# IlzeAmandaA/VAE-GP-ODE

Measured on AMD Instinct MI355X. Metric: latent_trajectories_per_sec, higher is better.
Workload: dtype f32; 1 GPU; configs[1]: ode1 DF q=6 M=100 S=256 T=16 batch=256; step = full ELBO training step (encoder, GP draw, rk4 rollout, decoder, ELBO, backward, Adam), L=1; global_batch=256, mc_draws=1, solver=rk4 (3/8 rule), parallelism=dp1, hip_graph=True, graph_scope=whole, gp_side_stream=True, batchnorm=per-process statistics

## Files before the change

vae-gp-ode_amd/csrc/gp_backward.hip:

```cpp
#include "gp_rollout.hpp"

namespace gp {

template <int DI, int DO, int NJ>
__device__ __forceinline__ void store_grads_rbf(const typename RbfTeamEval<DI, DO, NJ>::Grads& G, float* __restrict__ out, int M, int S,
                                                int wave, int lane, float (*sInd)[64][4 * RbfLayout<DI, DO>::RQ2],
                                                float (*sUni)[((DO + 1) / 2) * DI]);
template <int D, int NJ, int PART = 0>
__device__ __forceinline__ void store_grads_df(const typename DfTeamEval<D, NJ>::Grads& G, float* __restrict__ out, int M, int S, int wave,
                                               int lane, float (*sInd)[64][4 * DfLayout<D>::RQ2],
                                               float (*sUni)[2 * D * ((D + 1) / 2) + (D + 1) / 2]);

template <class EV, bool PG> struct GradsOf { using type = NoGrads; };
template <class EV> struct GradsOf<EV, true> { using type = typename EV::Grads; };

template <class EV, int DI, int DO, int ORDER, int METHOD, bool PG = false, bool SUB = false>
__global__ __launch_bounds__(64 * EV::kTeam) void rollout_bwd_team_kernel(const float* __restrict__ pack, int M, int S,
                                                                const float* __restrict__ xstage, const float* __restrict__ gzt,
                                                                const float* __restrict__ ts, int N, int T,
                                                                float* __restrict__ gz0, float* __restrict__ astage, Draws dw,
                                                                float* __restrict__ slab = nullptr, size_t pack_floats = 0) {
  constexpr int NS = stages_of(METHOD);
  __shared__ float slots[2 * EV::kTeam * TeamCombine::DP];
  pack += blockIdx.y * dw.pack; xstage += blockIdx.y * dw.in; gzt += blockIdx.y * dw.in2; gz0 += blockIdx.y * dw.out; astage += blockIdx.y * dw.out2;
  const int lane = threadIdx.x & 63, wave = threadIdx.x >> 6;
  EV ev;
  ev.init(pack, M, S, slots, wave, lane);
  using GR = typename GradsOf<EV, PG>::type;
  GR G;
  if constexpr (PG) G.zero();
  const float third = (float)(1.0 / 3.0);
  const int sub = sub_count<SUB>(dw.sub);
  for (int n = blockIdx.x; n < N; n += gridDim.x) {
    const float* gz = gzt + (size_t)n * T * DI;
    const float* xs = xstage + (size_t)n * (T - 1) * sub * NS * DI;
    float* as = astage + (size_t)n * (T - 1) * sub * NS * DO;
    float lam[DI];
#pragma unroll
    for (int i = 0; i < DI; ++i) lam[i] = gz[(size_t)(T - 1) * DI + i];
    const float* tn = ts_row(ts, n, dw.ts);
    for (int t = T - 2; t >= 0; --t) {
      const float dt = sub_step<SUB>(tn[t], tn[t + 1], sub);
      for (int r = (t + 1) * sub - 1; r >= t * sub; --r) {
        const float* xt = xs + (size_t)r * NS * DI;
        float* at = as + (size_t)r * NS * DO;
        float x[DI], g[DI], af[DO];
        if (METHOD == 0) {
          float a1[DI];
#pragma unroll
          for (int i = 0; i < DI; ++i) { a1[i] = dt * lam[i]; x[i] = xt[i]; }
          ode_vjp<EV, DI, DO, ORDER, GR>(ev, x, a1, g, af, &G);
          if (wave == 0) store_state<DO>(at, af, lane);
#pragma unroll
          for (int i = 0; i < DI; ++i) lam[i] += g[i];
        } else if (METHOD == 2) {
          float a1[DI], a2[DI], ay[DI];
#pragma unroll
          for (int i = 0; i < DI; ++i) { a2[i] = dt * lam[i]; x[i] = xt[DI + i]; }
          ode_vjp<EV, DI, DO, ORDER, GR>(ev, x, a2, g, af, &G);
          if (wave == 0) store_state<DO>(at + DO, af, lane);
#pragma unroll
          for (int i = 0; i < DI; ++i) { ay[i] = lam[i] + g[i]; a1[i] = 0.5f * dt * g[i]; x[i] = xt[i]; }
          ode_vjp<EV, DI, DO, ORDER, GR>(ev, x, a1, g, af, &G);
          if (wave == 0) store_state<DO>(at, af, lane);
#pragma unroll
          for (int i = 0; i < DI; ++i) lam[i] = ay[i] + g[i];
        } else {
          float a1[DI], a2[DI], a3[DI], a4[DI], ay[DI];
#pragma unroll
          for (int i = 0; i < DI; ++i) {
            const float l8 = lam[i] * dt * 0.125f;
            a1[i] = l8; a4[i] = l8; a2[i] = 3.f * l8; a3[i] = 3.f * l8; ay[i] = lam[i];
          }
#pragma unroll
          for (int i = 0; i < DI; ++i) x[i] = xt[3 * DI + i];
          ode_vjp<EV, DI, DO, ORDER, GR>(ev, x, a4, g, af, &G);
          if (wave == 0) store_state<DO>(at + 3 * DO, af, lane);
#pragma unroll
          for (int i = 0; i < DI; ++i) { ay[i] += g[i]; a1[i] += dt * g[i]; a2[i] -= dt * g[i]; a3[i] += dt * g[i]; }
#pragma unroll
          for (int i = 0; i < DI; ++i) x[i] = xt[2 * DI + i];
          ode_vjp<EV, DI, DO, ORDER, GR>(ev, x, a3, g, af, &G);
// ... 176 lines not shown
    float red[NU];
    wave_sum_all<NU>(flat, red);
    if (lane == 0) {
#pragma unroll
      for (int e = 0; e < NU; ++e) sUni[wave][e] = red[e];
    }
  }
  __syncthreads();
  if (half == 0 && j < MJ) {
    float* ind_out = out + 4 * L::rff_f4(S);
    float v[4 * L::RQ2];
#pragma unroll
    for (int q = 0; q < 4 * L::RQ2; ++q) v[q] = G.ind[q] + sInd[j][lane][q];
#pragma unroll
    for (int q = 0; q < L::RQ2; ++q) st4(ind_out, (size_t)(j * L::RQ2 + q) * 64 + lane, &v[4 * q]);
  }
  {
    float* uni_out = out + 4 * (L::rff_f4(S) + L::ind_f4(M));
    const int t = threadIdx.x;
    if (t < D * D) {
      const int a = t / D, b = t % D, h = b / DH, bb = b % DH;
      uni_out[a * D + b] = sUni[h][a * DH + bb] + sUni[h + 2][a * DH + bb];
      uni_out[D * D + a * D + b] = sUni[h][D * DH + a * DH + bb] + sUni[h + 2][D * DH + a * DH + bb];
    }
    if (t < D) {
      const int h = t / DH, bb = t % DH;
      uni_out[2 * D * D + t] = sUni[h][2 * D * DH + bb] + sUni[h + 2][2 * D * DH + bb];
    }
  }
}

template <int D, int NJ>
__global__ __launch_bounds__(256) void param_grad_df_kernel(const float* __restrict__ pack, int M, int S,
                                                             const float* __restrict__ xr, const float* __restrict__ ar,
                                                             int R, int rows_per_chunk, float* __restrict__ slab,
                                                             size_t pack_floats, int prior_only, Draws dw, int slab_chunks) {
  pack += blockIdx.y * dw.pack; xr += blockIdx.y * dw.in; ar += blockIdx.y * dw.in2; slab += (size_t)blockIdx.y * slab_chunks * pack_floats;
  using EV = DfTeamEval<D, NJ>;
  using L = DfLayout<D>;
  constexpr int DH = (D + 1) / 2;
  constexpr int NU = 2 * D * DH + DH;
  __shared__ float slots[2 * TEAM * TeamCombine::DP];
  __shared__ __attribute__((aligned(16))) float sInd[2][64][4 * L::RQ2];
  __shared__ float sUni[TEAM][NU];
  const int lane = threadIdx.x & 63, wave = threadIdx.x >> 6;
  EV ev;
  ev.init(pack, M, S, slots, wave, lane);
  typename EV::Grads G;
  G.zero();
  const int r0 = blockIdx.x * rows_per_chunk;
  const int r1 = min(R, r0 + rows_per_chunk);
  for (int r = r0; r < r1; ++r) {
    float x[D], a[D];
#pragma unroll
    for (int i = 0; i < D; ++i) { x[i] = xr[(size_t)r * D + i]; a[i] = ar[(size_t)r * D + i]; }
    ev.grad_row(x, a, G, prior_only != 0);
  }
  store_grads_df<D, NJ>(G, slab + (size_t)blockIdx.x * pack_floats, M, S, wave, lane, sInd, sUni);
}

template <int D, int PART>
__device__ __forceinline__ void pgrad_df_part(const float* __restrict__ pack, int M, int S, const float* __restrict__ xr,
                                              const float* __restrict__ ar, int r0, int r1, float* __restrict__ out, int prior_only) {
  using EV = DfTeamEval<D, 1>;
  using L = DfLayout<D>;
  constexpr int DH = (D + 1) / 2;
  constexpr int NU = 2 * D * DH + DH;
  __shared__ float slots[2 * TEAM * TeamCombine::DP];
  __shared__ __attribute__((aligned(16))) float sInd[2][64][4 * L::RQ2];
  __shared__ float sUni[TEAM][NU];
  const int lane = threadIdx.x & 63, wave = threadIdx.x >> 6;
  EV ev;
  ev.init(pack, M, S, slots, wave, lane);
  typename EV::Grads G;
  G.zero();
  for (int r = r0; r < r1; ++r) {
    float x[D], a[D];
#pragma unroll
    for (int i = 0; i < D; ++i) { x[i] = xr[(size_t)r * D + i]; a[i] = ar[(size_t)r * D + i]; }
    ev.template grad_row_part<PART>(x, a, G, prior_only != 0);
  }
  store_grads_df<D, 1, PART>(G, out, M, S, wave, lane, sInd, sUni);
}
template <int D>
__global__ __launch_bounds__(256, 2) void param_grad_df_split_kernel(const float* __restrict__ pack, int M, int S,
                                                                      const float* __restrict__ xr, const float* __restrict__ ar,
                                                                      int R, int rows_per_chunk, float* __restrict__ slab,
                                                                      size_t pack_floats, int prior_only, Draws dw, int slab_chunks) {
  pack += blockIdx.y * dw.pack; xr += blockIdx.y * dw.in; ar += blockIdx.y * dw.in2; slab += (size_t)blockIdx.y * slab_chunks * pack_floats;
  const int r0 = blockIdx.x * rows_per_chunk, r1 = min(R, r0 + rows_per_chunk);
  float* out = slab + (size_t)blockIdx.x * pack_floats;
  if (blockIdx.z == 0) pgrad_df_part<D, 1>(pack, M, S, xr, ar, r0, r1, out, prior_only);
  else pgrad_df_part<D, 2>(pack, M, S, xr, ar, r0, r1, out, prior_only);
}

template <int DI, int DO>
__global__ __launch_bounds__(256) void param_grad_rbf_stream_kernel(const float* __restrict__ pack, int M, int S,
                                                                     const float* __restrict__ xr, const float* __restrict__ ar,
                                                                     int R, int rows_per_chunk, float* __restrict__ slab,
                                                                     size_t pack_floats, int prior_only, Draws dw, int slab_chunks) {
  pack += blockIdx.y * dw.pack; xr += blockIdx.y * dw.in; ar += blockIdx.y * dw.in2; slab += (size_t)blockIdx.y * slab_chunks * pack_floats;
  using L = RbfLayout<DI, DO>;
  constexpr int DH = (DO + 1) / 2;
  __shared__ __attribute__((aligned(16))) float sInd[2][64][4 * L::RQ2];
  __shared__ float sUni[TEAM][DH * DI];
  const int lane = threadIdx.x & 63, wave = __builtin_amdgcn_readfirstlane(threadIdx.x >> 6);
  const float4* p4 = reinterpret_cast<const float4*>(pack);
  const float4* i4 = p4 + L::rff_f4(S);
  const float* wl = pack + 4 * (L::rff_f4(S) + L::ind_f4(M));
  const int r0 = blockIdx.x * rows_per_chunk, r1 = min(R, r0 + rows_per_chunk);
  float* out = slab + (size_t)blockIdx.x * pack_floats;
  const int SJ = cdiv(S, 64), MJ = cdiv(M, 64);
  for (int rec = wave; rec < SJ * DO; rec += TEAM) {
    float4 rq[L::RQ];
    load_record<L::RQ>(p4, rec, lane, rq);
    float g[4 * L::RQ];
#pragma unroll
    for (int q = 0; q < 4 * L::RQ; ++q) g[q] = 0.f;
    const int d = rec % DO;
    for (int r = r0; r < r1; ++r) {
      float x[DI], gx[DI];
#pragma unroll
      for (int i = 0; i < DI; ++i) { x[i] = xr[(size_t)r * DI + i]; gx[i] = 0.f; }
      rbf_rff_bwd<DI, DO, true>(rq, x, ar[(size_t)r * DO + d], gx, g);
    }
#pragma unroll
    for (int q = 0; q < L::RQ; ++q) st4(out, ((size_t)rec * L::RQ + q) * 64 + lane, &g[4 * q]);
  }
  const int half = wave & 1;
  float gwl[DH][DI];
#pragma unroll
  for (int d = 0; d < DH; ++d)
#pragma unroll
    for (int i = 0; i < DI; ++i) gwl[d][i] = 0.f;
  float* ind_out = out + 4 * L::rff_f4(S);
  for (int jb = 0; jb < MJ; jb += 2) {
    const int j = jb + (wave >> 1);
    const bool valid = j < MJ;
    float4 ind[L::RQ2];
    float gi[4 * L::RQ2];
#pragma unroll
    for (int q = 0; q < 4 * L::RQ2; ++q) gi[q] = 0.f;
    if (valid) {
      load_record<L::RQ2>(i4, j, lane, ind);
      if (!prior_only) {
        for (int r = r0; r < r1; ++r) {
          asm volatile("" ::: "memory");
          float x[DI], a[DO], gx[DI];
#pragma unroll
          for (int i = 0; i < DI; ++i) { x[i] = xr[(size_t)r * DI + i]; gx[i] = 0.f; }
#pragma unroll
          for (int i = 0; i < DO; ++i) a[i] = ar[(size_t)r * DO + i];
          rbf_ind_half_bwd<DI, DO, true>(ind, x, wl, half, a, gx, gi, gwl);
        }
      }
    }
    if (half == 1) {
#pragma unroll
      for (int q = 0; q < 4 * L::RQ2; ++q) sInd[wave >> 1][lane][q] = gi[q];
    }
    __syncthreads();
    if (half == 0 && valid) {
      float v[4 * L::RQ2];
#pragma unroll
      for (int q = 0; q < 4 * L::RQ2; ++q) v[q] = gi[q] + sInd[wave >> 1][lane][q];
#pragma unroll
      for (int q = 0; q < L::RQ2; ++q) st4(ind_out, ((size_t)j * L::RQ2 + q) * 64 + lane, &v[4 * q]);
    }
    __syncthreads();
  }
  {
    float flat[DH * DI], red[DH * DI];
#pragma unroll
    for (int e = 0; e < DH * DI; ++e) flat[e] = gwl[e / DI][e % DI];
    wave_sum_all<DH * DI>(flat, red);
    if (lane == 0) {
// ... 46 lines not shown
    for (int q = 0; q < L::RQ; ++q) st4(out, ((size_t)rec * L::RQ + q) * 64 + lane, &g[4 * q]);
  }
  const int part = wave % NP, slot = wave / NP;
  float gwab[D][DQ], gil2[D][DQ], gvar[DQ];
#pragma unroll
  for (int a = 0; a < D; ++a)
#pragma unroll
    for (int b = 0; b < DQ; ++b) { gwab[a][b] = 0.f; gil2[a][b] = 0.f; }
#pragma unroll
  for (int b = 0; b < DQ; ++b) gvar[b] = 0.f;
  float* ind_out = out + 4 * L::rff_f4(S);
  for (int jb = 0; jb < MJ; jb += RPI) {
    const int j = jb + slot;
    const bool valid = j < MJ;
    float4 ind[L::RQ2];
    float gi[4 * L::RQ2];
#pragma unroll
    for (int q = 0; q < 4 * L::RQ2; ++q) gi[q] = 0.f;
    if (valid) {
      load_record<L::RQ2>(i4, j, lane, ind);
      if (!prior_only) {
        for (int r = r0; r < r1; ++r) {
          asm volatile("" ::: "memory");
          float x[D], a[D], gx[D];
#pragma unroll
          for (int i = 0; i < D; ++i) { x[i] = xr[(size_t)r * D + i]; a[i] = ar[(size_t)r * D + i]; gx[i] = 0.f; }
          df_ind_part_bwd<D, NP, true>(ind, x, uni, part, a, gx, gi, gwab, gil2, gvar);
        }
      }
    }
    if (part > 0) {
#pragma unroll
      for (int q = 0; q < 4 * L::RQ2; ++q) sInd[slot][part - 1][lane][q] = gi[q];
    }
    __syncthreads();
    if (part == 0 && valid) {
      float v[4 * L::RQ2];
#pragma unroll
      for (int q = 0; q < 4 * L::RQ2; ++q) {
        v[q] = gi[q];
#pragma unroll
        for (int pp = 0; pp < NP - 1; ++pp) v[q] += sInd[slot][pp][lane][q];
      }
#pragma unroll
      for (int q = 0; q < L::RQ2; ++q) st4(ind_out, ((size_t)j * L::RQ2 + q) * 64 + lane, &v[4 * q]);
    }
    __syncthreads();
  }
  {
    float flat[NU];
#pragma unroll
    for (int a = 0; a < D; ++a)
#pragma unroll
      for (int b = 0; b < DQ; ++b) { flat[a * DQ + b] = gwab[a][b]; flat[D * DQ + a * DQ + b] = gil2[a][b]; }
#pragma unroll
    for (int b = 0; b < DQ; ++b) flat[2 * D * DQ + b] = gvar[b];
    float red[NU];
    wave_sum_all<NU>(flat, red);
    if (lane == 0) {
#pragma unroll
      for (int e = 0; e < NU; ++e) sUni[wave][e] = red[e];
    }
  }
  __syncthreads();
  {
    float* uni_out = out + 4 * (L::rff_f4(S) + L::ind_f4(M));
    for (int t = threadIdx.x; t < D * D; t += 256) {
      const int a = t / D, b = t % D, pt = b / DQ, bb = b % DQ;
      float v0 = 0.f, v1 = 0.f;
      for (int w = pt; w < TEAM; w += NP) { v0 += sUni[w][a * DQ + bb]; v1 += sUni[w][D * DQ + a * DQ + bb]; }
      uni_out[a * D + b] = v0;
      uni_out[D * D + a * D + b] = v1;
    }
    if (threadIdx.x < D) {
      const int t = threadIdx.x, pt = t / DQ, bb = t % DQ;
      float v = 0.f;
      for (int w = pt; w < TEAM; w += NP) v += sUni[w][2 * D * DQ + bb];
      uni_out[2 * D * D + t] = v;
    }
  }
}

__global__ __launch_bounds__(1024) void reduce_slab_kernel(const float* __restrict__ slab, int nchunk, size_t pack_floats,
                                                            float* __restrict__ gpack, int accumulate, size_t gpack_dstride, int slab_chunks) {
  __shared__ float red[16][64];
  slab += (size_t)blockIdx.y * slab_chunks * pack_floats; gpack += blockIdx.y * gpack_dstride;
  const int ex = threadIdx.x & 63, cg = threadIdx.x >> 6;
  const size_t e = (size_t)blockIdx.x * 64 + ex;
  float acc = 0.f;
  if (e < pack_floats) {
#pragma unroll 8
    for (int c = cg; c < nchunk; c += 16) acc += slab[(size_t)c * pack_floats + e];
  }
  red[cg][ex] = acc;
  __syncthreads();
  if (cg == 0 && e < pack_floats) {
    float v = accumulate ? gpack[e] : 0.f;
#pragma unroll
    for (int g = 0; g < 16; ++g) v += red[g][ex];
    gpack[e] = v;
  }
}

static Draws rollout_bwd_draws(int method, int Di, int Do, const RolloutBwdArgs& a, int nd, size_t pack_floats) {
  const size_t rows = record_rows(a.N, a.T, a.substeps, method);
  Draws d;
  d.nd = nd; d.pack = pack_floats;
  d.in = rows * Di; d.in2 = (size_t)a.N * a.T * Di;
  d.out = (size_t)a.N * Di; d.out2 = rows * Do;
  d.ts = a.ts_per_traj ? (size_t)a.T : 0; d.sub = a.substeps;
  return d;
}

int rollout_bwd(int kernel, int order, int method, int Di, int Do, const RolloutBwdArgs& a, int nd, hipStream_t st) {
  static const char* const who = "gpode_rollout_bwd";
  static const char* const tags[2][2] = {{"rollout_bwd_rbf", "rollout_bwd_rbf_stream"}, {"rollout_bwd_df", "rollout_bwd_df_stream"}};
  size_t pf = 0;
  if (cache_sizes(kernel, Di, Do, a.M, a.S, &pf, nullptr)) return 1;
  if (method < 0 || method > 2) return set_error("gpode_rollout_bwd: method %d (0 euler, 1 rk4, 2 midpoint; 3 dopri5: gpode_rollout_adaptive_bwd_n)", method);
  if (kernel != 0 && order != 1) return set_error("gpode_rollout_bwd: DF kernel is first-order only");
  const Draws dw = rollout_bwd_draws(method, Di, Do, a, nd, pf);
  return dispatch_dims(who, kernel, Di, Do, [&](auto k, auto di, auto dO) {
    constexpr int KERNEL = decltype(k)::value, DI = decltype(di)::value, DO = decltype(dO)::value;
    return dispatch_order<DI, DO>(who, order, [&](auto o) {
      return dispatch_method(method, [&](auto m) {
        constexpr int ORDER = decltype(o)::value, METHOD = decltype(m)::value;
        return reverse_route<KERNEL, DI, DO>(a.N, a.M, a.S, [&](auto ev, const LaunchGeom& g) {
          using EV = typename decltype(ev)::type;
          return dispatch_substeps(dw.sub, [&](auto sb) {
            if (launch_route(rollout_bwd_team_kernel<EV, DI, DO, ORDER, METHOD, false, decltype(sb)::value>, g, nd, st, a.pack, a.M, a.S, a.xstage,
                             a.gzt, a.ts, a.N, a.T, a.gz0, a.astage, dw, (float*)nullptr, (size_t)0))
              return 1;
            return check_launch(tags[KERNEL][g.route]);
          });
        });
      });
    });
  });
}

#define GP_PGRAD_RBF_DIMS(X) X(6) X(4) X(2) X(3)
template <class F> static int pgrad_width(int kernel, int Do, F&& f) {
  if (kernel == 0) {
#define X(d) if (Do == d) return f(int_c<d>{});
    GP_PGRAD_RBF_DIMS(X)
#undef X
  }
  return 0;
}
int rollout_bwd_pgrad_chunks(int kernel, int order, int method, int Di, int Do, int M, int S, int N) {
  if (order != 1 || Di != Do || (method != 0 && method != 1) || N < 1) return 0;
  return pgrad_width(kernel, Do, [&](auto d) { return rbf_team_ok<decltype(d)::value, decltype(d)::value>(M, S) ? team_grid(N) : 0; });
}
int rollout_bwd_pgrad(int kernel, int order, int method, int Di, int Do, const RolloutBwdArgs& a, int nd, hipStream_t st) {
  size_t pf = 0;
  if (cache_sizes(kernel, Di, Do, a.M, a.S, &pf, nullptr)) return 1;
  const int grid = rollout_bwd_pgrad_chunks(kernel, order, method, Di, Do, a.M, a.S, a.N);
  if (grid == 0) return set_error("gpode_rollout_bwd_pgrad: no fused form for kernel=%d order=%d method=%d Di=%d Do=%d M=%d S=%d", kernel, order,
                                  method, Di, Do, a.M, a.S);
  if (a.nchunk != grid) return set_error("gpode_rollout_bwd_pgrad: slab for %d chunks, the launch has %d", a.nchunk, grid);
  const Draws dw = rollout_bwd_draws(method, Di, Do, a, nd, pf);
  const LaunchGeom g{kRouteTeam, grid, 256, 0};
  const int done = pgrad_width(kernel, Do, [&](auto d) {
    constexpr int D = decltype(d)::value;
    const auto sweep = [&](auto m) {
      return dispatch_substeps(dw.sub, [&](auto sb) {
        return launch_route(rollout_bwd_team_kernel<RbfTeamEval<D, D, 1>, D, D, 1, decltype(m)::value, true, decltype(sb)::value>, g, nd, st,
                            a.pack, a.M, a.S, a.xstage, a.gzt, a.ts, a.N, a.T, a.gz0, a.astage, dw, a.slab, pf);
      });
    };
    if (method == 0) sweep(int_c<0>{});
    else sweep(int_c<1>{});
    return 1;
  });
  if (!done) return set_error("gpode_rollout_bwd_pgrad: width %d not built", Do);
  if (check_launch("rollout_bwd_pgrad")) return 1;
  hipLaunchKernelGGL(reduce_slab_kernel, dim3((unsigned)((pf + 63) / 64), nd), 1024, 0, st, a.slab, grid, pf, a.gpack, 0, pf, grid);
  return check_launch("reduce_slab");
}

int rhs_vjp(int kernel, int Di, int Do, int M, int S, const float* pack, const float* x, const float* a, int R, float* gx,
            int prior_only, hipStream_t st, Draws dw) {
  static const char* const tags[2][2] = {{"rhs_vjp_rbf", "rhs_vjp_rbf_stream"}, {"rhs_vjp_df", "rhs_vjp_df_stream"}};
  if (R <= 0) return 0;
  return dispatch_dims("gpode_rhs_vjp", kernel, Di, Do, [&](auto k, auto di, auto dO) {
    constexpr int KERNEL = decltype(k)::value, DI = decltype(di)::value, DO = decltype(dO)::value;
    return reverse_route<KERNEL, DI, DO>(R, M, S, [&](auto ev, const LaunchGeom& g) {
      using EV = typename decltype(ev)::type;
      if (launch_route(rhs_vjp_team_kernel<EV, DI, DO>, g, dw.nd, st, pack, M, S, x, a, R, gx, prior_only, dw)) return 1;
      return check_launch(tags[KERNEL][g.route]);
    });
  });
}

template <int DI, int DO>
static int launch_pgrad_rbf(const float* pack, int M, int S, const float* xr, const float* ar, int R, int rpc, int used, float* slab,
                            size_t pf, int prior_only, hipStream_t st, Draws dw, int nchunk) {
  if constexpr (DO <= 8) {
    if (rbf_team_ok<DI, DO>(M, S)) {
      hipLaunchKernelGGL((param_grad_rbf_kernel<DI, DO, 1>), dim3(used, dw.nd), 256, 0, st, pack, M, S, xr, ar, R, rpc, slab, pf, prior_only, dw, nchunk);
      return check_launch("param_grad_rbf");
    }
  }
  hipLaunchKernelGGL((param_grad_rbf_stream_kernel<DI, DO>), dim3(used, dw.nd), 256, 0, st, pack, M, S, xr, ar, R, rpc, slab, pf, prior_only, dw, nchunk);
  return check_launch("param_grad_rbf_stream");
}

template <int D>
static int launch_pgrad_df(const float* pack, int M, int S, const float* xr, const float* ar, int R, int rpc, int used, float* slab,
                           size_t pf, int prior_only, hipStream_t st, Draws dw, int nchunk) {
  if constexpr (D <= 8) {
    if (df_team_ok<D>(M, S)) {
      if constexpr (D == 6) {
        if (R >= 1024) {
          hipLaunchKernelGGL((param_grad_df_split_kernel<D>), dim3(used, dw.nd, 2), 256, 0, st, pack, M, S, xr, ar, R, rpc, slab, pf, prior_only, dw, nchunk);
          return check_launch("param_grad_df_split");
        }
      }
      hipLaunchKernelGGL((param_grad_df_kernel<D, 1>), dim3(used, dw.nd), 256, 0, st, pack, M, S, xr, ar, R, rpc, slab, pf, prior_only, dw, nchunk);
      return check_launch("param_grad_df");
    }
  }
  hipLaunchKernelGGL((param_grad_df_stream_kernel<D, (D > 8 ? 4 : 2)>), dim3(used, dw.nd), 256, 0, st, pack, M, S, xr, ar, R, rpc, slab, pf, prior_only, dw, nchunk);
  return check_launch("param_grad_df_stream");
}

int param_grad(int kernel, int Di, int Do, int M, int S, const float* pack, const float* xr, const float* ar, int R,
               float* slab, int nchunk, float* gpack, int accumulate, int prior_only, hipStream_t st, Draws dw) {
  size_t pf = 0;
  if (cache_sizes(kernel, Di, Do, M, S, &pf, nullptr)) return 1;
  if (R <= 0 || nchunk <= 0) return set_error("gpode_param_grad: R=%d nchunk=%d", R, nchunk);
  const int rpc = cdiv(R, nchunk);
  const int used = cdiv(R, rpc);
  const int rc = dispatch_dims("gpode_param_grad", kernel, Di, Do, [&](auto k, auto di, auto dO) {
    constexpr int DI = decltype(di)::value, DO = decltype(dO)::value;
    if constexpr (decltype(k)::value == 0) return launch_pgrad_rbf<DI, DO>(pack, M, S, xr, ar, R, rpc, used, slab, pf, prior_only, st, dw, nchunk);
    else return launch_pgrad_df<DO>(pack, M, S, xr, ar, R, rpc, used, slab, pf, prior_only, st, dw, nchunk);
  });
  if (rc) return rc;
  const char* route = *last_launch_slot();
  hipLaunchKernelGGL(reduce_slab_kernel, dim3((unsigned)((pf + 63) / 64), dw.nd), 1024, 0, st, slab, used, pf, gpack, accumulate, dw.out, nchunk);
  if (check_launch("reduce_slab")) return 1;
  *last_launch_slot() = route;
  return 0;
}

}
```

vae-gp-ode_amd/csrc/gp_eval.hpp:

```cpp
#pragma once
#include <hip/hip_runtime.h>
#include "wave_reduce.hpp"

#define GP_WAVE 64
#define GP_LOG2E 1.4426950408889634f
#define GP_INV2PI 0.15915494309189535f

namespace gp {

__host__ __device__ constexpr int cdiv(int a, int b) { return (a + b - 1) / b; }

template <int DI, int DO> struct RbfLayout {
  static constexpr int RQ = cdiv(DI + 2, 4);
  static constexpr int RQ2 = cdiv(DI + DO, 4);
  __host__ __device__ static size_t rff_f4(int S) { return (size_t)cdiv(S, 64) * DO * RQ * 64; }
  __host__ __device__ static size_t ind_f4(int M) { return (size_t)cdiv(M, 64) * RQ2 * 64; }
  __host__ __device__ static size_t uni_floats() { return (size_t)cdiv(DO * DI, 4) * 4; }
  __host__ __device__ static size_t total_floats(int M, int S) { return 4 * (rff_f4(S) + ind_f4(M)) + uni_floats(); }
};

template <int D> struct DfLayout {
  static constexpr int RQ = cdiv(2 * D + 3, 4);
  static constexpr int RQ2 = cdiv(2 * D, 4);
  __host__ __device__ static size_t rff_f4(int S) { return (size_t)cdiv(S, 64) * D * RQ * 64; }
// ... 220 lines not shown
#pragma unroll
  for (int k = 0; k < D; ++k) t = fmaf(x[k], f[k], t);
  t = __builtin_amdgcn_fractf(t);
  const float c = __builtin_amdgcn_cosf(t), sn = __builtin_amdgcn_sinf(t);
  float A = 0.f;
#pragma unroll
  for (int j = 0; j < D; ++j) A = fmaf(a[j], f[D + 3 + j], A);
  const float rt = GP_2PI * fmaf(f[D + 2], c, -f[D + 1] * sn);
  const float coef = A * rt;
#pragma unroll
  for (int k = 0; k < D; ++k) gx[k] = fmaf(coef, f[k], gx[k]);
  if (WITH_G) {
    const float rr = fmaf(f[D + 2], sn, f[D + 1] * c);
#pragma unroll
    for (int k = 0; k < D; ++k) g[k] = fmaf(coef, x[k], g[k]);
#pragma unroll
    for (int j = 0; j < D; ++j) g[D + 3 + j] = fmaf(a[j], rr, g[D + 3 + j]);
  }
}

template <int D, bool WITH_G>
__device__ __forceinline__ void df_ind_half_bwd(const float4 (&r)[DfLayout<D>::RQ2], const float (&x)[D],
                                                const float* __restrict__ uni, int half, const float (&a)[D],
                                                float (&gx)[D], float (&g)[4 * DfLayout<D>::RQ2],
                                                float (&gwab)[D][(D + 1) / 2], float (&gil2)[D][(D + 1) / 2],
                                                float (&gvar)[(D + 1) / 2]) {
  constexpr int DH = (D + 1) / 2;
  float f[4 * DfLayout<D>::RQ2];
  unpack(r, f);
  const float* wab = uni;
  const float* il2 = uni + D * D;
  const float* var = uni + 2 * D * D;
  float dl[D];
  float r2 = 0.f;
#pragma unroll
  for (int q = 0; q < D; ++q) { dl[q] = x[q] - f[q]; r2 = fmaf(dl[q], dl[q], r2); }
  const int b0 = half * DH;
  float gd[D];
  float gr2 = 0.f;
#pragma unroll
  for (int q = 0; q < D; ++q) gd[q] = 0.f;
#pragma unroll
  for (int bb = 0; bb < DH; ++bb) {
    const bool hi_ok = DH + bb < D;
    const int bidx = b0 + bb < D ? b0 + bb : D - 1;
    const bool live = half ? hi_ok : true;
    const float dlb = half ? (hi_ok ? dl[hi_ok ? DH + bb : 0] : 0.f) : dl[bb];
    const float ab = live ? (half ? (hi_ok ? a[hi_ok ? DH + bb : 0] : 0.f) : a[bb]) : 0.f;
    const float vb = var[bidx];
    float gdb = 0.f;
    float gv = 0.f;
#pragma unroll
    for (int aa = 0; aa < D; ++aa) {
      const float il = il2[aa * D + bidx], wv = wab[aa * D + bidx];
      const float E = exp2_fast(r2 * wv);
      const bool diag = (aa == bidx);
      const float term = dl[aa] * dlb * il + (diag ? ((float)(D - 1) - r2 * il) : 0.f);
      const float G = ab * f[D + aa];
      const float GE = G * vb * E * il;
      gr2 = fmaf(GE, term * (GP_LN2 * wv) - (diag ? il : 0.f), gr2);
      gd[aa] = fmaf(GE * il, dlb, gd[aa]);
      gdb = fmaf(GE * il, dl[aa], gdb);
      if (WITH_G) {
        g[D + aa] = fmaf(ab, vb * E * il * term, g[D + aa]);
        gv = fmaf(G, E * il * term, gv);
        gwab[aa][bb] = fmaf(G * vb * il * term, E * GP_LN2 * r2, gwab[aa][bb]);
        gil2[aa][bb] = fmaf(G * vb * E, term + il * (dl[aa] * dlb - (diag ? r2 : 0.f)), gil2[aa][bb]);
      }
    }
    if (WITH_G) gvar[bb] += gv;
    if (live) {
      if (half) { if (hi_ok) gd[hi_ok ? DH + bb : 0] += gdb; }
      else gd[bb] += gdb;
    }
  }
#pragma unroll
  for (int q = 0; q < D; ++q) {
    const float v = fmaf(2.f * gr2, dl[q], gd[q]);
    gx[q] += v;
    if (WITH_G) g[q] -= v;
  }
}

}
```

vae-gp-ode_amd/csrc/gp_team.hpp:

```cpp
#pragma once
#include "gp_eval.hpp"

namespace gp {

constexpr int TEAM = 4;

template <int TS> struct TeamCombineT {
  static constexpr int DP = 16;
  float* slots;
  int wave, lane, parity;
  __device__ __forceinline__ void init(float* s, int w, int l) { slots = s; wave = w; lane = l; parity = 0; }
  template <int NV> __device__ __forceinline__ void run(const float (&part)[NV], float (&f)[NV]) {
    static_assert(NV <= DP, "slot too small");
    float* mine = slots + (parity * TS + wave) * DP;
    if (lane == 0) {
#pragma unroll
      for (int d = 0; d < NV; ++d) mine[d] = part[d];
    }
    __syncthreads();
    const float* base = slots + parity * TS * DP;
#pragma unroll
    for (int d = 0; d < NV; ++d) {
      float v = base[d];
#pragma unroll
// ... 107 lines not shown
  TeamCombine comb;
  static __host__ bool fits(int M, int S) { return cdiv(S, 64) <= TEAM * NJ && cdiv(M, 64) * 2 <= TEAM; }
  __device__ __forceinline__ void init(const float* pack, int M, int S, float* lds, int wave, int lane) {
    const float4* p4 = reinterpret_cast<const float4*>(pack);
    const int SJ = cdiv(S, 64), MJ = cdiv(M, 64);
    const float4 z = make_float4(0.f, 0.f, 0.f, 0.f);
#pragma unroll
    for (int jn = 0; jn < NJ; ++jn) {
      const int j = wave + TEAM * jn;
#pragma unroll
      for (int i = 0; i < D; ++i)
#pragma unroll
        for (int q = 0; q < L::RQ; ++q) rff[jn * D + i][q] = j < SJ ? p4[((j * D + i) * L::RQ + q) * 64 + lane] : z;
    }
    const float4* i4 = p4 + L::rff_f4(S);
    const int j = wave >> 1;
    half = wave & 1;
#pragma unroll
    for (int q = 0; q < L::RQ2; ++q) ind[q] = j < MJ ? i4[(j * L::RQ2 + q) * 64 + lane] : z;
    uni = pack + 4 * (L::rff_f4(S) + L::ind_f4(M));
    comb.init(lds, wave, lane);
  }
  template <int MODE> __device__ __forceinline__ void eval(const float (&x)[D], float (&f)[D]) {
    float acc[D];
#pragma unroll
    for (int d = 0; d < D; ++d) acc[d] = 0.f;
    if (MODE != 2) {
#pragma unroll
      for (int r = 0; r < NJ * D; ++r) df_rff_record<D>(rff[r], x, acc);
    }
    if (MODE != 1) df_ind_record_half<D>(ind, x, uni, half, acc);
    float part[D];
    wave_sum_all<D>(acc, part);
    comb.run<D>(part, f);
  }
  __device__ __forceinline__ void vjp(const float (&x)[D], const float (&a)[D], float (&gx)[D], bool prior_only = false) {
    float acc[D];
#pragma unroll
    for (int i = 0; i < D; ++i) acc[i] = 0.f;
    float g0[4 * L::RQ], g1[4 * L::RQ2], g2[D][(D + 1) / 2], g3[D][(D + 1) / 2], g4[(D + 1) / 2];
#pragma unroll
    for (int r = 0; r < NJ * D; ++r) df_rff_bwd<D, false>(rff[r], x, a, acc, g0);
    if (!prior_only) df_ind_half_bwd<D, false>(ind, x, uni, half, a, acc, g1, g2, g3, g4);
    float part[D];
    wave_sum_all<D>(acc, part);
    comb.run<D>(part, gx);
  }
  struct Grads {
    float rff[NJ * D][4 * L::RQ];
    float ind[4 * L::RQ2];
    float gwab[D][(D + 1) / 2], gil2[D][(D + 1) / 2], gvar[(D + 1) / 2];
    __device__ __forceinline__ void zero() {
#pragma unroll
      for (int r = 0; r < NJ * D; ++r)
#pragma unroll
        for (int q = 0; q < 4 * L::RQ; ++q) rff[r][q] = 0.f;
#pragma unroll
      for (int q = 0; q < 4 * L::RQ2; ++q) ind[q] = 0.f;
#pragma unroll
      for (int a = 0; a < D; ++a)
#pragma unroll
        for (int b = 0; b < (D + 1) / 2; ++b) { gwab[a][b] = 0.f; gil2[a][b] = 0.f; }
#pragma unroll
      for (int b = 0; b < (D + 1) / 2; ++b) gvar[b] = 0.f;
    }
  };
  __device__ __forceinline__ void grad_row(const float (&x)[D], const float (&a)[D], Grads& G, bool prior_only) const {
    float gx[D];
#pragma unroll
    for (int i = 0; i < D; ++i) gx[i] = 0.f;
#pragma unroll
    for (int r = 0; r < NJ * D; ++r) df_rff_bwd<D, true>(rff[r], x, a, gx, G.rff[r]);
    if (!prior_only) df_ind_half_bwd<D, true>(ind, x, uni, half, a, gx, G.ind, G.gwab, G.gil2, G.gvar);
  }
  template <int PART> __device__ __forceinline__ void grad_row_part(const float (&x)[D], const float (&a)[D], Grads& G, bool prior_only) const {
    float gx[D];
#pragma unroll
    for (int i = 0; i < D; ++i) gx[i] = 0.f;
    if constexpr (PART != 2) {
#pragma unroll
      for (int r = 0; r < NJ * D; ++r) df_rff_bwd<D, true>(rff[r], x, a, gx, G.rff[r]);
    }
    if constexpr (PART != 1) {
      if (!prior_only) df_ind_half_bwd<D, true>(ind, x, uni, half, a, gx, G.ind, G.gwab, G.gil2, G.gvar);
    }
  }
  __device__ __forceinline__ void vjp_grad(const float (&x)[D], const float (&a)[D], float (&gx)[D], Grads& G) {
    float acc[D];
#pragma unroll
    for (int i = 0; i < D; ++i) acc[i] = 0.f;
#pragma unroll
    for (int r = 0; r < NJ * D; ++r) df_rff_bwd<D, true>(rff[r], x, a, acc, G.rff[r]);
    df_ind_half_bwd<D, true>(ind, x, uni, half, a, acc, G.ind, G.gwab, G.gil2, G.gvar);
    float part[D];
    wave_sum_all<D>(acc, part);
    comb.run<D>(part, gx);
  }
};

template <int NQ>
__device__ __forceinline__ void load_record(const float4* __restrict__ base, int rec, int lane, float4 (&r)[NQ]) {
#pragma unroll
  for (int q = 0; q < NQ; ++q) r[q] = base[((size_t)rec * NQ + q) * 64 + lane];
}

template <int N> __device__ __forceinline__ float pick(const float (&v)[N], int idx) {
  float r = v[0];
#pragma unroll
  for (int i = 1; i < N; ++i) r = (idx == i) ? v[i] : r;
  return r;
}

template <int D, int NP, bool WITH_G>
__device__ __forceinline__ void df_ind_part_bwd(const float4 (&r)[DfLayout<D>::RQ2], const float (&x)[D],
                                                const float* __restrict__ uni, int part, const float (&a)[D],
                                                float (&gx)[D], float (&g)[4 * DfLayout<D>::RQ2],
                                                float (&gwab)[D][(D + NP - 1) / NP], float (&gil2)[D][(D + NP - 1) / NP],
                                                float (&gvar)[(D + NP - 1) / NP]) {
  constexpr int DQ = (D + NP - 1) / NP;
  float f[4 * DfLayout<D>::RQ2];
  unpack(r, f);
  const float* wab = uni;
  const float* il2 = uni + D * D;
  const float* var = uni + 2 * D * D;
  float dl[D];
  float r2 = 0.f;
#pragma unroll
  for (int q = 0; q < D; ++q) { dl[q] = x[q] - f[q]; r2 = fmaf(dl[q], dl[q], r2); }
  float gd[D];
  float gr2 = 0.f;
#pragma unroll
  for (int q = 0; q < D; ++q) gd[q] = 0.f;
#pragma unroll
  for (int bb = 0; bb < DQ; ++bb) {
    const int b = part * DQ + bb;
    const bool live = b < D;
    const int bidx = live ? b : D - 1;
    const float dlb = live ? pick<D>(dl, bidx) : 0.f;
    const float ab = live ? pick<D>(a, bidx) : 0.f;
    const float vb = var[bidx];
    float gdb = 0.f, gv = 0.f;
#pragma unroll
    for (int aa = 0; aa < D; ++aa) {
      const float il = il2[aa * D + bidx], wv = wab[aa * D + bidx];
      const float E = exp2_fast(r2 * wv);
      const bool diag = (aa == bidx);
      const float term = dl[aa] * dlb * il + (diag ? ((float)(D - 1) - r2 * il) : 0.f);
      const float G = ab * f[D + aa];
      const float GE = G * vb * E * il;
      gr2 = fmaf(GE, term * (GP_LN2 * wv) - (diag ? il : 0.f), gr2);
      gd[aa] = fmaf(GE * il, dlb, gd[aa]);
      gdb = fmaf(GE * il, dl[aa], gdb);
      if (WITH_G) {
        g[D + aa] = fmaf(ab, vb * E * il * term, g[D + aa]);
        gv = fmaf(G, E * il * term, gv);
        gwab[aa][bb] = fmaf(G * vb * il * term, E * GP_LN2 * r2, gwab[aa][bb]);
        gil2[aa][bb] = fmaf(G * vb * E, term + il * (dl[aa] * dlb - (diag ? r2 : 0.f)), gil2[aa][bb]);
      }
    }
    if (WITH_G) gvar[bb] += gv;
#pragma unroll
    for (int q = 0; q < D; ++q) gd[q] += (live && q == bidx) ? gdb : 0.f;
  }
#pragma unroll
  for (int q = 0; q < D; ++q) {
    const float v = fmaf(2.f * gr2, dl[q], gd[q]);
    gx[q] += v;
// ... 141 lines not shown
```

Before: 109,300 trajectories/s.

## Balance DF param-grad split kernel work and specialize inducing-half backward

The D=6 split parameter-gradient kernel used to give the RFF part and the inducing part the same number of row chunks. It now gives them different chunk counts, weighted 5:17 toward the heavier inducing part, and uses a packed slab layout that the reduce kernel reads with a two-region stride. The inducing backward is also specialized at compile time per half role, chosen by a wave-uniform branch, which removes the runtime half predication. The risks are a slab capacity fallback, a fixed weight ratio that may not fit other shapes, and extra code size.

```diff
diff --git a/vae-gp-ode_amd/csrc/gp_backward.hip b/vae-gp-ode_amd/csrc/gp_backward.hip
--- a/vae-gp-ode_amd/csrc/gp_backward.hip
+++ b/vae-gp-ode_amd/csrc/gp_backward.hip
@@ -1,3 +1,4 @@
+#include <algorithm>
 #include "gp_rollout.hpp"
 
 namespace gp {
@@ -340,16 +341,26 @@
   }
   store_grads_df<D, 1, PART>(G, out, M, S, wave, lane, sInd, sUni);
 }
+struct SplitChunks {
+  int n1, rpc1, n2, rpc2;
+  size_t rff;
+};
 template <int D>
 __global__ __launch_bounds__(256, 2) void param_grad_df_split_kernel(const float* __restrict__ pack, int M, int S,
                                                                       const float* __restrict__ xr, const float* __restrict__ ar,
-                                                                      int R, int rows_per_chunk, float* __restrict__ slab,
+                                                                      int R, SplitChunks sc, float* __restrict__ slab,
                                                                       size_t pack_floats, int prior_only, Draws dw, int slab_chunks) {
   pack += blockIdx.y * dw.pack; xr += blockIdx.y * dw.in; ar += blockIdx.y * dw.in2; slab += (size_t)blockIdx.y * slab_chunks * pack_floats;
-  const int r0 = blockIdx.x * rows_per_chunk, r1 = min(R, r0 + rows_per_chunk);
-  float* out = slab + (size_t)blockIdx.x * pack_floats;
-  if (blockIdx.z == 0) pgrad_df_part<D, 1>(pack, M, S, xr, ar, r0, r1, out, prior_only);
-  else pgrad_df_part<D, 2>(pack, M, S, xr, ar, r0, r1, out, prior_only);
+  const int b = __builtin_amdgcn_readfirstlane(blockIdx.x);
+  if (b < sc.n1) {
+    const int r0 = b * sc.rpc1, r1 = min(R, r0 + sc.rpc1);
+    pgrad_df_part<D, 1>(pack, M, S, xr, ar, r0, r1, slab + (size_t)b * sc.rff, prior_only);
+  } else {
+    const int c = b - sc.n1;
+    const int r0 = c * sc.rpc2, r1 = min(R, r0 + sc.rpc2);
+    float* part2 = slab + (size_t)sc.n1 * sc.rff + (size_t)c * (pack_floats - sc.rff);
+    pgrad_df_part<D, 2>(pack, M, S, xr, ar, r0, r1, part2 - sc.rff, prior_only);
+  }
 }
 
 template <int DI, int DO>
@@ -562,15 +573,22 @@
 }
 
 __global__ __launch_bounds__(1024) void reduce_slab_kernel(const float* __restrict__ slab, int nchunk, size_t pack_floats,
-                                                            float* __restrict__ gpack, int accumulate, size_t gpack_dstride, int slab_chunks) {
+                                                            float* __restrict__ gpack, int accumulate, size_t gpack_dstride, int slab_chunks,
+                                                            size_t split = 0, int nchunk2 = 0) {
   __shared__ float red[16][64];
   slab += (size_t)blockIdx.y * slab_chunks * pack_floats; gpack += blockIdx.y * gpack_dstride;
   const int ex = threadIdx.x & 63, cg = threadIdx.x >> 6;
   const size_t e = (size_t)blockIdx.x * 64 + ex;
+  size_t off = e, stride = pack_floats;
+  if (split > 0) {
+    const bool lo = (size_t)blockIdx.x * 64 < split;
+    if (!lo) { slab += (size_t)nchunk * split; off = e - split; nchunk = nchunk2; }
+    stride = lo ? split : pack_floats - split;
+  }
   float acc = 0.f;
   if (e < pack_floats) {
 #pragma unroll 8
-    for (int c = cg; c < nchunk; c += 16) acc += slab[(size_t)c * pack_floats + e];
+    for (int c = cg; c < nchunk; c += 16) acc += slab[(size_t)c * stride + off];
   }
   red[cg][ex] = acc;
   __syncthreads();
@@ -686,14 +704,38 @@
   return check_launch("param_grad_rbf_stream");
 }
 
+#ifndef GPODE_PGRAD_BALANCE
+#define GPODE_PGRAD_BALANCE 1
+#endif
+static SplitChunks split_chunks(int R, int used, int nchunk, size_t pf, size_t rff) {
+  constexpr int W1 = 5, W2 = 17;
+  const auto chunks = [&](int n1, int n2) {
+    SplitChunks s;
+    s.rpc1 = cdiv(R, n1); s.n1 = cdiv(R, s.rpc1);
+    s.rpc2 = cdiv(R, n2); s.n2 = cdiv(R, s.rpc2);
+    s.rff = rff;
+    return s;
+  };
+  const SplitChunks even = chunks(used, used);
+  if (!GPODE_PGRAD_BALANCE) return even;
+  const int total = 2 * used;
+  int n2 = (int)(((long long)total * W2 + (W1 + W2) / 2) / (W1 + W2));
+  n2 = std::max(1, std::min(std::min(n2, total - 1), R));
+  const int n1 = std::max(1, std::min(total - n2, R));
+  const SplitChunks s = chunks(n1, n2);
+  return s.n1 * rff + s.n2 * (pf - rff) <= (size_t)nchunk * pf ? s : even;
+}
+
 template <int D>
 static int launch_pgrad_df(const float* pack, int M, int S, const float* xr, const float* ar, int R, int rpc, int used, float* slab,
-                           size_t pf, int prior_only, hipStream_t st, Draws dw, int nchunk) {
+                           size_t pf, int prior_only, hipStream_t st, Draws dw, int nchunk, SplitChunks* split) {
   if constexpr (D <= 8) {
     if (df_team_ok<D>(M, S)) {
       if constexpr (D == 6) {
         if (R >= 1024) {
-          hipLaunchKernelGGL((param_grad_df_split_kernel<D>), dim3(used, dw.nd, 2), 256, 0, st, pack, M, S, xr, ar, R, rpc, slab, pf, prior_only, dw, nchunk);
+          const SplitChunks sc = split_chunks(R, used, nchunk, pf, 4 * DfLayout<D>::rff_f4(S));
+          hipLaunchKernelGGL((param_grad_df_split_kernel<D>), dim3(sc.n1 + sc.n2, dw.nd), 256, 0, st, pack, M, S, xr, ar, R, sc, slab, pf, prior_only, dw, nchunk);
+          *split = sc;
           return check_launch("param_grad_df_split");
         }
       }
@@ -712,14 +754,16 @@
   if (R <= 0 || nchunk <= 0) return set_error("gpode_param_grad: R=%d nchunk=%d", R, nchunk);
   const int rpc = cdiv(R, nchunk);
   const int used = cdiv(R, rpc);
+  SplitChunks split{};
   const int rc = dispatch_dims("gpode_param_grad", kernel, Di, Do, [&](auto k, auto di, auto dO) {
     constexpr int DI = decltype(di)::value, DO = decltype(dO)::value;
     if constexpr (decltype(k)::value == 0) return launch_pgrad_rbf<DI, DO>(pack, M, S, xr, ar, R, rpc, used, slab, pf, prior_only, st, dw, nchunk);
-    else return launch_pgrad_df<DO>(pack, M, S, xr, ar, R, rpc, used, slab, pf, prior_only, st, dw, nchunk);
+    else return launch_pgrad_df<DO>(pack, M, S, xr, ar, R, rpc, used, slab, pf, prior_only, st, dw, nchunk, &split);
   });
   if (rc) return rc;
   const char* route = *last_launch_slot();
-  hipLaunchKernelGGL(reduce_slab_kernel, dim3((unsigned)((pf + 63) / 64), dw.nd), 1024, 0, st, slab, used, pf, gpack, accumulate, dw.out, nchunk);
+  hipLaunchKernelGGL(reduce_slab_kernel, dim3((unsigned)((pf + 63) / 64), dw.nd), 1024, 0, st, slab, split.n1 ? split.n1 : used, pf, gpack, accumulate,
+                     dw.out, nchunk, split.n1 ? split.rff : (size_t)0, split.n2);
   if (check_launch("reduce_slab")) return 1;
   *last_launch_slot() = route;
   return 0;
diff --git a/vae-gp-ode_amd/csrc/gp_eval.hpp b/vae-gp-ode_amd/csrc/gp_eval.hpp
--- a/vae-gp-ode_amd/csrc/gp_eval.hpp
+++ b/vae-gp-ode_amd/csrc/gp_eval.hpp
@@ -326,4 +326,66 @@
   }
 }
 
-}
+template <int D, int HALF, bool WITH_G>
+__device__ __forceinline__ void df_ind_role_bwd(const float4 (&r)[DfLayout<D>::RQ2], const float (&x)[D],
+                                                const float* __restrict__ uni, const float (&a)[D],
+                                                float (&gx)[D], float (&g)[4 * DfLayout<D>::RQ2],
+                                                float (&gwab)[D][(D + 1) / 2], float (&gil2)[D][(D + 1) / 2],
+                                                float (&gvar)[(D + 1) / 2]) {
+  constexpr int DH = (D + 1) / 2;
+  float f[4 * DfLayout<D>::RQ2];
+  unpack(r, f);
+  const float* wab = uni;
+  const float* il2 = uni + D * D;
+  const float* var = uni + 2 * D * D;
+  float dl[D];
+  float r2 = 0.f;
+#pragma unroll
+  for (int q = 0; q < D; ++q) { dl[q] = x[q] - f[q]; r2 = fmaf(dl[q], dl[q], r2); }
+  float gd[D];
+  float gr2 = 0.f;
+#pragma unroll
+  for (int q = 0; q < D; ++q) gd[q] = 0.f;
+#pragma unroll
+  for (int bb = 0; bb < DH; ++bb) {
+    constexpr int b0 = HALF * DH;
+    if (b0 + bb < D) {
+      const int b = b0 + bb < D ? b0 + bb : 0;
+      const float dlb = dl[b];
+      const float ab = a[b];
+      const float vb = var[b];
+      float gdb = 0.f;
+      float gv = 0.f;
+#pragma unroll
+      for (int aa = 0; aa < D; ++aa) {
+        const float il = il2[aa * D + b], wv = wab[aa * D + b];
+        const float E = exp2_fast(r2 * wv);
+        const bool diag = (aa == b);
+        float term = dl[aa] * dlb * il;
+        if (diag) term += (float)(D - 1) - r2 * il;
+        const float G = ab * f[D + aa];
+        const float GE = G * vb * E * il;
+        gr2 = diag ? fmaf(GE, term * (GP_LN2 * wv) - il, gr2) : fmaf(GE, term * (GP_LN2 * wv), gr2);
+        gd[aa] = fmaf(GE * il, dlb, gd[aa]);
+        gdb = fmaf(GE * il, dl[aa], gdb);
+        if (WITH_G) {
+          g[D + aa] = fmaf(ab, vb * E * il * term, g[D + aa]);
+          gv = fmaf(G, E * il * term, gv);
+          gwab[aa][bb] = fmaf(G * vb * il * term, E * GP_LN2 * r2, gwab[aa][bb]);
+          gil2[aa][bb] = diag ? fmaf(G * vb * E, term + il * (dl[aa] * dlb - r2), gil2[aa][bb])
+                              : fmaf(G * vb * E, fmaf(il, dl[aa] * dlb, term), gil2[aa][bb]);
+        }
+      }
+      if (WITH_G) gvar[bb] += gv;
+      gd[b] += gdb;
+    }
+  }
+#pragma unroll
+  for (int q = 0; q < D; ++q) {
+    const float v = fmaf(2.f * gr2, dl[q], gd[q]);
+    gx[q] += v;
+    if (WITH_G) g[q] -= v;
+  }
+}
+
+}
diff --git a/vae-gp-ode_amd/csrc/gp_team.hpp b/vae-gp-ode_amd/csrc/gp_team.hpp
--- a/vae-gp-ode_amd/csrc/gp_team.hpp
+++ b/vae-gp-ode_amd/csrc/gp_team.hpp
@@ -213,7 +213,10 @@
       for (int r = 0; r < NJ * D; ++r) df_rff_bwd<D, true>(rff[r], x, a, gx, G.rff[r]);
     }
     if constexpr (PART != 1) {
-      if (!prior_only) df_ind_half_bwd<D, true>(ind, x, uni, half, a, gx, G.ind, G.gwab, G.gil2, G.gvar);
+      if (!prior_only) {
+        if (__builtin_amdgcn_readfirstlane(half)) df_ind_role_bwd<D, 1, true>(ind, x, uni, a, gx, G.ind, G.gwab, G.gil2, G.gvar);
+        else df_ind_role_bwd<D, 0, true>(ind, x, uni, a, gx, G.ind, G.gwab, G.gil2, G.gvar);
+      }
     }
   }
   __device__ __forceinline__ void vjp_grad(const float (&x)[D], const float (&a)[D], float (&gx)[D], Grads& G) {
```

Measured after the change: 110,200 trajectories/s (median of 6 runs). About the same (+0.9%).
